# martenlienen/generative-turbulence

Hardware: AMD Instinct MI355X
Metric: U-Net fwd+bwd voxels/sec (DDPM training step, 192x64x48x4) (higher is better)
Workload: dtype bf16

## Files before the change

generative-turbulence_amd/csrc/tdx_conv3.h:

```cpp
#pragma once
#include "tdx_common.h"

struct Conv3Geom {
    int B;
    int Xi, Yi, Zi;
    int Xo, Yo, Zo;
    int off;
};

bool conv3_mfma_supported(int C1, int C2, int Cout);
bool conv3_mfma_f32_supported(int C1, int C2, int Cout);
static inline int conv3_layout_kc(int dtype, int K, int N) {
    if (dtype == 1 || dtype == 3) return conv3_mfma_supported(K, 0, N) ? 16 : 0;
    return conv3_mfma_f32_supported(K, 0, N) ? 8 : 0;
}
static inline bool conv3_uses_mfma_layout(int dtype, int K, int N) { return (dtype == 1 || dtype == 3) && conv3_mfma_supported(K, 0, N); }
bool conv3_mfma_split_supported(int C1, int C2, int Cout);

struct Conv3Ext {
    int ld1, ld2;
    const void* init;
    bool init_shared;
};

// ... 45 lines not shown

int conv3_mfma_launch(const Conv3Call& c);
int conv3_mfma_split_launch(const Conv3Call& c);
int conv3_mfma_f32_launch(const Conv3Call& c);
int conv3_direct_launch(const Conv3Call& c);
int conv3_fold_launch(const Conv3Call& c);

int conv3_ring_depth(int C1, int C2, int N, int B, int X, int Y, int Z, bool data_gradient);
int conv3_ring_launch(const Conv3Call& c, int depth);

bool conv3_small_plan(Conv3SmallPlan& p, int C1, int C2, int N, int B, int X, int Y, int Z, bool data_gradient, bool split);
int conv3_small_launch(const Conv3Call& c, const Conv3SmallPlan& p);

struct Conv3WgradCall {
    const void* x1; int C1;
    const void* x2; int C2;
    const void* dy;
    float* dwp;
    float* dbias;
    int B, X, Y, Z, Cout;
    hipStream_t st;
    float* slabs; int max_slabs; int* nslab;
    bool hf;
};
bool tdx_deterministic();
static inline float* conv3_wgrad_merge(const Conv3WgradCall& c, int& nsplit, int64_t& slab_stride) {
    if (tdx_deterministic() && c.slabs != nullptr && nsplit > c.max_slabs) nsplit = c.max_slabs > 0 ? c.max_slabs : 1;
    const bool use_slabs = c.slabs != nullptr && nsplit <= c.max_slabs;
    slab_stride = use_slabs ? (int64_t)27 * (c.C1 + c.C2) * c.Cout : 0;
    if (c.nslab) *c.nslab = use_slabs ? nsplit : 0;
    return use_slabs ? c.slabs : c.dwp;
}
bool conv3_wgrad_mfma_supported(int C1, int C2, int Cout);
bool conv3_wgrad_mfma_split_supported(int C1, int C2, int Cout);
bool conv3_wgrad_mfma_f32_supported(int C1, int C2, int Cout);
int conv3_wgrad_mfma_launch(const Conv3WgradCall& c);
int conv3_wgrad_small_launch(const Conv3WgradCall& c);
int conv3_wgrad_ring_launch(const Conv3WgradCall& c);
int conv3_wgrad_mfma_split_launch(const Conv3WgradCall& c);
int conv3_wgrad_split_ring_launch(const Conv3WgradCall& c);
int conv3_wgrad_mfma_f32_launch(const Conv3WgradCall& c);
int conv3_wgrad_direct_launch(const Conv3WgradCall& c, int dtype);
int conv3_unpack_wgrad_launch(const Conv3WgradCall& c, float* dw, float* dbw, float* dbias, bool many);
int tdx_persistent_cus();
int ordered_sum_launch(const float* slabs, int nslab, int64_t stride, float* dst, int rows, int cols, int64_t ld, bool add,
                       hipStream_t st);
size_t bias_grad_ordered_scratch_floats(int C);
int bias_grad_ordered_launch(const void* dy, int64_t nvox, int C, int dtype, float* dbias, float* part, size_t part_floats,
                             hipStream_t st);
void* tdx_scratch_ptr();
size_t tdx_scratch_bytes();

size_t conv3_shell_buffer_bytes(int B, int X, int Y, int Z, int N);
int conv3_shell_launch(const void* dy, const void* wb, void* d1, int D1, void* d2, int B, int X, int Y, int Z, int K, int N,
                       int mode, hipStream_t st, void* sbuf = nullptr);

#define TDX_GN_REPLICAS 32
int gn_finalize_launch(double* acc, float* stats, int B, int C, int G, int64_t V, float eps, int replicas,
                       hipStream_t st);
int gn_stats_launch(const void* x, float* stats, int B, int64_t V, int C, int G, float eps, int dtype, void* workspace,
                    bool clean, hipStream_t stream);
```

generative-turbulence_amd/csrc/tdx_conv3_entry.hip:

```cpp
#include "tdx_common.h"
#include "tdx_conv3.h"
#include <stdlib.h>
#include <algorithm>

int tdx_persistent_cus() {
    const char* env = getenv("TDX_PERSISTENT_CUS");
    int n = env ? atoi(env) : 256;
    n = n < 8 ? 8 : (n > 256 ? 256 : n);
    return n & ~7;
}
static void* g_scratch = nullptr;
static size_t g_scratch_bytes = 0;
void* tdx_scratch_ptr() { return g_scratch; }
size_t tdx_scratch_bytes() { return g_scratch_bytes; }
extern "C" int tdx_set_scratch(void* ptr, size_t bytes) {
    if (ptr != nullptr && bytes < 64) return TDX_EINVAL;
    g_scratch = ptr;
    g_scratch_bytes = ptr ? bytes : 0;
    return TDX_OK;
}

Conv3Route conv3_route(int dtype, int impl, int C1, int C2, int N, int B, int X, int Y, int Z, bool data_gradient) {
    Conv3Route r;
    r.fmt = dtype; r.family = TDX_KERNEL_DIRECT; r.status = TDX_OK; r.ring_depth = 0;
// ... 144 lines not shown
                                      const void* add1, const void* add2, int B, int X, int Y, int Z, int Cout, int dtype,
                                      int impl, void* workspace, void* stream) {
    return conv3_bwd_data_impl(dy, wb, dx1, C1, dx2, C2, add1, add2, B, X, Y, Z, Cout, dtype, impl, workspace, stream);
}

#define W3_MAX_SLABS 8
static int w3_slab_capacity(int Cin, int Cout) {
    const int64_t c = ((int64_t)1 << 19) / ((int64_t)Cin * Cout);
    return (int)(c < W3_MAX_SLABS ? W3_MAX_SLABS : (c > 512 ? 512 : c));
}
extern "C" size_t tdx_conv3_bwd_weight_workspace_bytes(int Cin, int Cout, int impl) {
    (void)impl;
    return (size_t)(1 + w3_slab_capacity(Cin, Cout)) * 27 * Cin * Cout * sizeof(float) + (size_t)Cout * sizeof(float) + 512;
}

struct Conv3WgradRoute {
    int (*launch)(const Conv3WgradCall&);
    bool f32;
    int status;
};
static Conv3WgradRoute conv3_wgrad_route(int dtype, int impl, int C1, int C2, int Cout) {
    if (dtype == TDX_F32 && impl == TDX_CONV_SPLIT && conv3_wgrad_mfma_split_supported(C1, C2, Cout))
        return {conv3_wgrad_mfma_split_launch, true, TDX_OK};
    if (dtype == TDX_F32 && impl != TDX_CONV_DIRECT && conv3_wgrad_mfma_f32_supported(C1, C2, Cout))
        return {conv3_wgrad_mfma_f32_launch, true, TDX_OK};
    if (impl == TDX_CONV_MFMA || (impl == TDX_CONV_AUTO && tdx_is_h16(dtype) && conv3_wgrad_mfma_supported(C1, C2, Cout))) {
        if (!tdx_is_h16(dtype)) return {nullptr, false, TDX_EDTYPE};
        if (!conv3_wgrad_mfma_supported(C1, C2, Cout)) return {nullptr, false, TDX_ESHAPE};
        return {conv3_wgrad_mfma_launch, false, TDX_OK};
    }
    return {nullptr, false, TDX_OK};
}

extern "C" int tdx_conv3_bwd_weight(const void* x1, int C1, const void* x2, int C2, const void* dy, float* dw,
                                    float* dbias, int B, int X, int Y, int Z, int Cout, int dtype, int impl,
                                    void* workspace, void* stream) {
    TDX_CHECK_ARG(x1 && dy && dw && workspace && B > 0 && X > 0 && Y > 0 && Z > 0 && C1 > 0 && C2 >= 0 && Cout > 0);
    TDX_CHECK_ARG(C2 == 0 || x2);
    const int Cin = C1 + C2;
    if ((C1 % 8) || (C2 % 8) || (Cout % 8)) return TDX_ESHAPE;
    hipStream_t st = as_stream(stream);
    const bool clean = (impl & TDX_WS_CLEAN) != 0;
    float* dwp = (float*)workspace;
    float* dbw = dwp + (size_t)27 * Cin * Cout;
    if (!clean) {
        int e = tdx_zero_async(dwp, ((size_t)27 * Cin * Cout + Cout) * sizeof(float), st);
        if (e != TDX_OK) return e;
    }
    const Conv3WgradRoute r = conv3_wgrad_route(dtype, impl & 0xff, C1, C2, Cout);
    if (r.status != TDX_OK) return r.status;
    int nslab = 0;
    const bool det = tdx_deterministic();
    float* slab_base = dbw + ((Cout + 63) / 64) * 64;
    auto ordered_bias = [&]() -> int {
        if (!det || !dbias) return TDX_OK;
        return bias_grad_ordered_launch(dy, (int64_t)B * X * Y * Z, Cout, dtype, dbias, slab_base,
                                        (size_t)W3_MAX_SLABS * 27 * Cin * Cout, st);
    };
    Conv3WgradCall c = {x1, C1, x2, C2, dy, dwp, (dbias && !det) ? dbw : nullptr, B, X, Y, Z, Cout, st, slab_base, 0, &nslab,
                        dtype == TDX_F16};
    if (r.launch != nullptr) {
        c.max_slabs = (r.f32 && !det) ? W3_MAX_SLABS : w3_slab_capacity(Cin, Cout);
    } else if (det) {
        c.max_slabs = std::min(w3_slab_capacity(Cin, Cout), 64);
    }
    const int rc = r.launch != nullptr ? r.launch(c) : conv3_wgrad_direct_launch(c, dtype);
// ... 5 lines not shown
```

generative-turbulence_amd/csrc/tdx_conv3_wgrad_mfma.hip:

```cpp
#include "tdx_conv3_wgrad.h"
#include <stdlib.h>

typedef WgradBrick<4> W3;
#define W3_NSTEPS (W3::NVOX / 16)
#define W3_TAPS_PER_WAVE 7

bool conv3_wgrad_mfma_supported(int C1, int C2, int Cout) {
    const bool c1_ok = (C1 % 32) == 0 || (C2 == 0 && (C1 % 16) == 0);
    return C1 > 0 && c1_ok && (C2 % 32) == 0 && (Cout % 32) == 0;
}

#ifdef W3_STAMPS
#define W3_NSTAMP 64
__device__ unsigned long long* w3_stamps_dev;
#define W3_T()                                                                              \
    do {                                                                                    \
        if (it_ >= 4 && it_ < 12) {                                                         \
            const unsigned long long t_ = __builtin_amdgcn_s_memtime();                     \
            if (lane == 0 && nst_ < W3_NSTAMP) sStamp_[wave * W3_NSTAMP + nst_] = t_;       \
            ++nst_;                                                                         \
        }                                                                                   \
    } while (0)
#else
#define W3_T() do { } while (0)
// ... 188 lines not shown
#endif

    const int r = lane & 31, hh = lane >> 5;
#pragma unroll
    for (int t = 0; t < W3_TAPS_PER_WAVE; ++t) {
        const int ltap = wave + 4 * t;
        if (ltap < 27) {
            const int tap = wgrad_global_tap(gv, ltap);
#pragma unroll
            for (int nt = 0; nt < NT; ++nt)
#pragma unroll
                for (int i = 0; i < 16; ++i) {
                    const int ci = ci0 + (i & 3) + 8 * (i >> 2) + 4 * hh;
                    if (ci >= Cin) continue;
                    float* dst = &dwp[((int64_t)tap * Cin + ci) * Cout + co0 + nt * 32 + r];
                    if (slab_stride) dst[(int64_t)split * slab_stride] = acc[t][nt][i];
                    else atomicAdd(dst, acc[t][nt][i]);
                }
        }
    }
    if (do_bias) {
        __syncthreads();
        float* red = reinterpret_cast<float*>(smem);
#pragma unroll
        for (int e = 0; e < 8; ++e) red[tid * 8 + e] = bs[e];
        __syncthreads();
        if (tid < 32 * NT) {
            const int q8 = tid >> 3, e = tid & 7;
            float t = 0.f;
            for (int k = q8; k < 256; k += 4 * NT) t += red[k * 8 + e];
            atomicAdd(&dbias[co0 + tid], t);
        }
    }
}

int conv3_wgrad_mfma_launch(const Conv3WgradCall& c) {
    const int Cout = c.Cout;
    {
        int rs = conv3_wgrad_small_launch(c);
        if (rs != TDX_ESHAPE) return rs;
#ifndef W3_STAMPS
        rs = conv3_wgrad_ring_launch(c);
        if (rs != TDX_ESHAPE) return rs;
#endif
    }
    const int Cin = c.C1 + c.C2;
    const int NT = (Cout % 64 == 0) ? 2 : 1;
    static const bool no_perm = getenv("TDX_CONV3_PERM") && atoi(getenv("TDX_CONV3_PERM")) == 0;
    WgradView g;
    const int nbricks = conv3_wgrad_view(g, c, W3::BX, W3::BY, W3::BZ, !no_perm);
    const int n_ci = (Cin + 31) / 32, n_co = Cout / (32 * NT);
    const int ntiles = n_ci * n_co;
    int nsplit = ((NT == 2 ? 256 : 512) + ntiles - 1) / ntiles;
    if (nsplit > nbricks) nsplit = nbricks;
    if (nsplit < 1) nsplit = 1;
    int64_t slab_stride;
    float* out = conv3_wgrad_merge(c, nsplit, slab_stride);
    size_t lds = W3::XBYTES + (size_t)NT * W3::GPLANE;
#ifdef W3_STAMPS
    lds += 4 * W3_NSTAMP * 8;
#endif
    dim3 grid((unsigned)(ntiles * nsplit));
#define W3_LAUNCH(NTV, HFV)                                                                                          \
    do {                                                                                                             \
        auto kern = conv3_wgrad_mfma_kernel<NTV, HFV>;                                                                  \
        hipError_t e = hipFuncSetAttribute((const void*)kern, hipFuncAttributeMaxDynamicSharedMemorySize, (int)lds); \
// ... 10 lines not shown
```

generative-turbulence_amd/csrc/tdx_conv3_wgrad_ring.hip:

```cpp
#include "tdx_conv3_wgrad.h"
#include <stdlib.h>
#include <algorithm>
#include <type_traits>

typedef WgradBrick<4> WR;
#define WR_NSTEPS (WR::NVOX / 16)
#define WR_XPIECES ((WR::NHALO * 4 + 63) / 64)
#define WR_XBUF (WR_XPIECES * 1024)
#define WR_XPW ((WR_XPIECES + 3) / 4)
#define WR_CW 8
#define WR_GBUF(NTN) ((NTN) * WR::GPLANE)
#define WR_GPW(NTN) (4 * (NTN))
#define WR_SLOTS(NTN) ((NTN) == 2 ? 7 : 4)

template <int NTN, bool HF>
__global__ void __launch_bounds__(768, 3)
conv3_wgrad_ring_kernel(const bf16* __restrict__ x1, int C1, const bf16* __restrict__ x2, int C2, const bf16* __restrict__ dy,
                        float* __restrict__ dwp, float* __restrict__ dbias, WgradView gv, int Cout, int nsplit, int n_ci_tiles,
                        int64_t slab_stride, const void* __restrict__ zeros) {
    extern __shared__ __attribute__((aligned(1024))) unsigned char smem[];
    unsigned char* sX = smem;
    unsigned char* sG = smem + 2 * WR_XBUF;
    constexpr int GBUF = WR_GBUF(NTN), GPW = WR_GPW(NTN), SLOTS = WR_SLOTS(NTN);
    const unsigned lds0 = lds_addr(smem);
// ... 159 lines not shown
                step(2 * s2 + 1, 1);
            }
        }
    };
    if (NTN == 2 ? odd : (cnt == 4 || bias_slot)) run(std::true_type{}); else run(std::false_type{});

    const int r = lane & 31, hh = lane >> 5;
#pragma unroll
    for (int i = 0; i < SLOTS; ++i) {
        const int T = first + i;
        if (i < cnt) {
            const int ltap = T / NTN, nt = T % NTN;
            const int tap = wgrad_global_tap(gv, ltap);
#pragma unroll
            for (int e = 0; e < 16; ++e) {
                const int ci = ci0 + (e & 3) + 8 * (e >> 2) + 4 * hh;
                if (ci >= Cin) continue;
                float* dst = &dwp[((int64_t)tap * Cin + ci) * Cout + co0 + nt * 32 + r];
                if (slab_stride) dst[(int64_t)split * slab_stride] = acc[i][e];
                else atomicAdd(dst, acc[i][e]);
            }
        } else if (bias_slot && i == SLOTS - 1 && dbias != nullptr && ci0 == 0 && hh == 0) {
            atomicAdd(&dbias[co0 + (NTN == 2 ? (wave - 6) * 32 : 0) + r], acc[i][0]);
        }
    }
}

bool conv3_wgrad_ring_supported(int C1, int C2, int Cout) {
    const char* env = getenv("TDX_WGRAD_RING");
    if (env && atoi(env) == 0) return false;
    return conv3_wgrad_mfma_supported(C1, C2, Cout) && (Cout % 32) == 0 && tdx_scratch_ptr() != nullptr && tdx_scratch_bytes() >= 16;
}

int conv3_wgrad_ring_launch(const Conv3WgradCall& c) {
    const int Cout = c.Cout;
    if (!conv3_wgrad_ring_supported(c.C1, c.C2, Cout)) return TDX_ESHAPE;
    const int Cin = c.C1 + c.C2;
    WgradView g;
    const int nbricks = conv3_wgrad_view(g, c, WR::BX, WR::BY, WR::BZ);
    const int NTN = (Cout % 64) == 0 ? 2 : 1;
    {
        const char* env = getenv("TDX_WGRAD_RING");
        if (NTN == 1 && env && atoi(env) == 2) return TDX_ESHAPE;
    }
    const int n_ci = (Cin + 31) / 32, n_co = Cout / (32 * NTN);
    const int ntiles = n_ci * n_co;
    const int cus = tdx_persistent_cus();
    int nsplit = cus >= 256 ? (256 + ntiles - 1) / ntiles : std::max(cus / ntiles, 1);
    if (nsplit > nbricks) nsplit = nbricks;
    if (nsplit < 1) nsplit = 1;
    if (nbricks < 4 * nsplit) return TDX_ESHAPE;
    const size_t lds = (size_t)2 * WR_XBUF + (size_t)2 * WR_GBUF(NTN);
    int64_t slab_stride;
    float* out = conv3_wgrad_merge(c, nsplit, slab_stride);
    static bool attr_set[2][2] = {{false, false}, {false, false}};
#define WR_GO(NTNV, HFV)                                                                                                          \
    do {                                                                                                                          \
        auto kern = conv3_wgrad_ring_kernel<NTNV, HFV>;                                                                           \
        if (!attr_set[NTNV - 1][HFV]) {                                                                                           \
            hipError_t e = hipFuncSetAttribute((const void*)kern, hipFuncAttributeMaxDynamicSharedMemorySize, (int)lds);          \
            if (e != hipSuccess) return (int)e;                                                                                   \
            attr_set[NTNV - 1][HFV] = true;                                                                                       \
        }                                                                                                                         \
        hipLaunchKernelGGL(kern, dim3((unsigned)(ntiles * nsplit)), dim3(768), lds, c.st, (const bf16*)c.x1, c.C1,                \
                           (const bf16*)c.x2, c.C2, (const bf16*)c.dy, out, c.dbias, g, Cout, nsplit, n_ci, slab_stride,          \
                           tdx_scratch_ptr());                                                                                    \
    } while (0)
    if (NTN == 2) { if (c.hf) WR_GO(2, true); else WR_GO(2, false); }
    else { if (c.hf) WR_GO(1, true); else WR_GO(1, false); }
#undef WR_GO
    return tdx_launch_status();
}
```

generative-turbulence_amd/csrc/tdx_conv3_wgrad_small.hip:

```cpp
#include "tdx_conv3_wgrad.h"
#include <stdlib.h>

#define WS_MAXROWS 256
#define WS_TAPS_PER_WAVE 7

struct WsGeom {
    int B, E[3];
    int nbg;
    int xs, gx;
    int Ix, Iy, Iz;
    int ngroups;
    int xbytes;
    int grows;
};

template <int NT, bool HF>
__global__ void __launch_bounds__(256, 1)
conv3_wgrad_small_kernel(const bf16* __restrict__ x1, int C1, const bf16* __restrict__ x2, int C2, const bf16* __restrict__ dy,
                         float* __restrict__ dwp, float* __restrict__ dbias, WsGeom g, int Cout, int nsplit, int n_ci_tiles,
                         int64_t slab_stride) {
    extern __shared__ __attribute__((aligned(16))) unsigned char smem[];
    const int gbytes = NT * g.grows * 64;
    unsigned char* sX = smem;
    unsigned char* sG = smem + 2 * g.xbytes;
// ... 136 lines not shown
            if (s + 1 < nsteps) {
                read_a(s3, A0);
                read_b(s2, B0);
                mfma_step(A1, B1);
                __builtin_amdgcn_sched_group_barrier(0x008, 1, 0);
                __builtin_amdgcn_sched_group_barrier(0x100, NRD, 0);
                __builtin_amdgcn_sched_group_barrier(0x008, NMF - 1, 0);
            }
        }
    }

    const int r = lane & 31, hh = lane >> 5;
#pragma unroll
    for (int t = 0; t < WS_TAPS_PER_WAVE; ++t) {
        const int tap = wave + 4 * t;
        if (tap < 27) {
#pragma unroll
            for (int nt = 0; nt < NT; ++nt)
#pragma unroll
                for (int i = 0; i < 16; ++i) {
                    const int ci = ci0 + (i & 3) + 8 * (i >> 2) + 4 * hh;
                    float* dst = &dwp[((int64_t)tap * Cin + ci) * Cout + co0 + nt * 32 + r];
                    if (slab_stride) dst[(int64_t)split * slab_stride] = acc[t][nt][i];
                    else atomicAdd(dst, acc[t][nt][i]);
                }
        }
    }
    if (do_bias && ones_slot && hh == 0) {
#pragma unroll
        for (int nt = 0; nt < NT; ++nt) atomicAdd(&dbias[co0 + nt * 32 + r], acc[WS_TAPS_PER_WAVE - 1][nt][0]);
    }
}

int conv3_wgrad_small_launch(const Conv3WgradCall& c) {
    const int B = c.B, X = c.X, Y = c.Y, Z = c.Z, Cout = c.Cout;
    static const int mode = getenv("TDX_WGRAD_SMALL") ? atoi(getenv("TDX_WGRAD_SMALL")) : 1;
    if (mode == 0) return TDX_ESHAPE;
    const int Cin = c.C1 + c.C2;
    if ((c.C1 % 32) || (c.C2 % 32) || (Cout % 32) || Cin < 128) return TDX_ESHAPE;
    const char* env_rows = getenv("TDX_WGRAD_SMALL_ROWS");
    const int64_t rows_total = (int64_t)B * X * Y * Z;
    if (rows_total > (env_rows ? atoi(env_rows) : 8000)) return TDX_ESHAPE;
    WsGeom g;
    g.B = B; g.E[0] = X; g.E[1] = Y; g.E[2] = Z;
    const int plane = Y * Z, V = X * plane;
    if (plane > WS_MAXROWS) return TDX_ESHAPE;
    if (V <= WS_MAXROWS) { g.nbg = std::min(B, WS_MAXROWS / V); g.xs = X; g.gx = 1; }
    else { g.nbg = 1; g.xs = WS_MAXROWS / plane; g.gx = ceil_div(X, g.xs); }
    g.Ix = g.xs + 2; g.Iy = Y + 2; g.Iz = Z + 2;
    const int NT = (Cout % 64 == 0) ? 2 : 1;
    auto sizes = [&]() {
        const int entries = g.nbg * g.Ix * g.Iy * g.Iz;
        g.xbytes = ((entries * 64 + 1023) >> 10) << 10;
        g.grows = ((g.nbg * g.xs * plane + 15) >> 4) << 4;
        return (size_t)2 * g.xbytes + (size_t)2 * NT * g.grows * 64 + (WS_MAXROWS + (g.xbytes >> 6)) * sizeof(unsigned);
    };
    size_t lds = sizes();
    while (lds > 160 * 1024 && (g.nbg > 1 || g.xs > 1)) {
        if (g.nbg > 1) --g.nbg; else { --g.xs; g.gx = ceil_div(X, g.xs); g.Ix = g.xs + 2; }
        lds = sizes();
    }
    if (lds > 160 * 1024) return TDX_ESHAPE;
    g.ngroups = ceil_div(B, g.nbg) * g.gx;
    const int n_ci = Cin / 32, n_co = Cout / (32 * NT);
    const int ntiles = n_ci * n_co;
    int nsplit = std::max(1, std::min(g.ngroups, ceil_div(256, ntiles)));
    int64_t slab_stride;
    float* out = conv3_wgrad_merge(c, nsplit, slab_stride);
    dim3 grid((unsigned)(ntiles * nsplit));
#define WS_LAUNCH(NTV, HFV)                                                                                           \
    do {                                                                                                              \
        auto kern = conv3_wgrad_small_kernel<NTV, HFV>;                                                               \
        static size_t attr = 0;                                                                                       \
        if (lds > attr) {                                                                                             \
            hipError_t e = hipFuncSetAttribute((const void*)kern, hipFuncAttributeMaxDynamicSharedMemorySize, (int)lds); \
            if (e != hipSuccess) return (int)e;                                                                       \
            attr = lds;                                                                                               \
        }                                                                                                             \
        hipLaunchKernelGGL(kern, grid, dim3(256), lds, c.st, (const bf16*)c.x1, c.C1, (const bf16*)c.x2, c.C2,        \
                           (const bf16*)c.dy, out, c.dbias, g, Cout, nsplit, n_ci, slab_stride);                      \
    } while (0)
    if (NT == 2) { if (c.hf) WS_LAUNCH(2, true); else WS_LAUNCH(2, false); }
    else { if (c.hf) WS_LAUNCH(1, true); else WS_LAUNCH(1, false); }
#undef WS_LAUNCH
    return tdx_launch_status();
}
```

generative-turbulence_amd/turbdiff_amd/_lib.py:

```python

from __future__ import annotations

import ctypes as C
import os
import threading
from pathlib import Path

import torch

_HERE = Path(__file__).resolve().parent
LIB_PATH = Path(os.environ.get("TDX_LIB", _HERE / "libtdx_hip.so"))

F32, BF16 = 0, 1
F16 = 3
CONV_AUTO, CONV_DIRECT, CONV_MFMA, CONV_SPLIT = 0, 1, 2, 3
F32_SPLIT = 2
WS_CLEAN = 0x100

_vp, _i, _i64, _u64, _f, _sz = C.c_void_p, C.c_int, C.c_int64, C.c_uint64, C.c_float, C.c_size_t

SIGNATURES = {
    "tdx_version": (_i, []),
    "tdx_arch": (C.c_char_p, []),
    "tdx_set_scratch": (_i, [_vp, _sz]),
    "tdx_ncv_to_nvc": (_i, [_vp, _vp, _i, _i, _i64, _i, _i, _vp]),
    "tdx_nvc_to_ncv": (_i, [_vp, _vp, _i, _i, _i64, _i, _i, _vp]),
    "tdx_cast": (_i, [_vp, _vp, _i64, _i, _i, _vp]),
    "tdx_conv3_pack_weight": (_i, [_vp, _vp, _vp, _i, _i, _i, _vp]),
    "tdx_conv3_pack_weights": (_i, [_vp, _i, _i, _vp]),
    "tdx_transpose_many": (_i, [_vp, _i, _vp]),
    "tdx_conv3_fwd": (_i, [_vp, _i, _vp, _i, _vp, _vp, _vp, _i, _i, _i, _i, _i, _i, _i, _vp]),
    "tdx_conv3_uses_ring": (_i, [_i] * 7),
    "tdx_conv3_ring_brick_depth": (_i, [_i] * 7),
    "tdx_conv3_fwd_kernel": (_i, [_i] * 9),
    "tdx_conv3_fwd_gn": (_i, [_vp, _i, _vp, _i, _vp, _vp, _vp, _vp, _i, _f, _vp, _i, _i, _i, _i, _i, _i, _i, _vp]),
    "tdx_conv3_fwd_partial": (_i, [_vp, _i, _i, _vp, _vp, _vp, _i, _vp, _vp, _i, _f, _vp, _i, _i, _i, _i, _i, _i, _i, _vp]),
    "tdx_conv3_bwd_data_workspace_bytes": (_sz, [_i, _i, _i, _i, _i, _i, _i]),
    "tdx_conv3_bwd_data": (_i, [_vp, _vp, _vp, _i, _vp, _i, _i, _i, _i, _i, _i, _i, _i, _i, _vp, _vp]),
    "tdx_conv3_bwd_data_add": (_i, [_vp, _vp, _vp, _i, _vp, _i, _vp, _vp, _i, _i, _i, _i, _i, _i, _i, _vp, _vp]),
    "tdx_conv3_bwd_weight_workspace_bytes": (_sz, [_i, _i, _i]),
    "tdx_conv3_bwd_weight": (_i, [_vp, _i, _vp, _i, _vp, _vp, _vp, _i, _i, _i, _i, _i, _i, _i, _vp, _vp]),
    "tdx_conv1_fwd": (_i, [_vp, _i, _vp, _i, _vp, _i, _vp, _vp, _vp, _i64, _i, _i, _vp]),
    "tdx_conv1_fwd_gn": (_i, [_vp, _i, _vp, _i, _vp, _i, _vp, _vp, _vp, _vp, _vp, _i, _vp, _i, _i64, _i, _i, _vp]),
    "tdx_conv1_bwd_weight": (_i, [_vp, _i, _vp, _i, _vp, _i, _vp, _i64, _i, _vp]),
    "tdx_conv1_bwd_weight_oc": (_i, [_vp, _i, _vp, _i, _vp, _i, _vp, _i, _i64, _i, _vp]),
    "tdx_encode_fwd": (_i, [_vp, _i, _vp, _vp, _vp, _i, _vp, _vp, _vp, _i, _i64, _i, _i, _vp]),
    "tdx_encode_bwd": (_i, [_vp, _vp, _i, _vp, _i, _vp, _vp, _vp, _vp, _vp, _vp, _i, _i64, _i, _i, _vp]),
    "tdx_decode_fwd": (_i, [_vp, _vp, _vp, _vp, _i, _i64, _i, _i, _i, _vp]),
    "tdx_decode_bwd": (_i, [_vp, _vp, _vp, _vp, _vp, _vp, _i, _i64, _i, _i, _i, _vp]),
    "tdx_gn_workspace_bytes": (_sz, [_i, _i]),
    "tdx_gn_stats": (_i, [_vp, _vp, _i, _i64, _i, _i, _f, _i, _vp, _vp]),
    "tdx_gn_apply": (_i, [_vp, _vp, _vp, _vp, _vp, _vp, _vp, _vp, _i, _i64, _i, _i, _i, _i, _vp]),
    "tdx_gn_apply_decode": (_i, [_vp, _vp, _vp, _vp, _vp, _vp, _vp, _vp, _i, _i64, _i, _i, _i, _i, _vp]),
    "tdx_gn_apply_encoded": (_i, [_vp, _vp, _vp, _vp, _vp, _i, _vp, _vp, _vp, _i, _vp, _vp, _vp, _i, _i64, _i, _i, _i, _vp]),
    "tdx_gn_bwd": (_i, [_vp] * 12 + [_i, _i64, _i, _i, _i, _i, _vp, _vp]),
    "tdx_resize_fwd": (_i, [_vp, _vp] + [_i] * 9 + [_vp]),
    "tdx_resize_bwd": (_i, [_vp, _vp, _vp] + [_i] * 9 + [_vp]),
    "tdx_attn_fwd": (_i, [_vp, _vp, _vp, _i, _i, _i, _i, _i, _vp]),
    "tdx_attn_bwd": (_i, [_vp, _vp, _vp, _vp, _vp, _i, _i, _i, _i, _i, _vp, _vp]),
    "tdx_attn_bwd_workspace_bytes": (_sz, [_i, _i, _i, _i]),
    "tdx_cell_mask": (_i, [_vp, _i64, _vp, _i64, _vp]),
    "tdx_q_sample": (_i, [_vp, _vp, _vp, _vp, _vp, _i, _vp, _i, _vp, _i, _i, _i64, _vp]),
    "tdx_p_sample_step": (_i, [_vp] * 7 + [_i, _vp, _i, _i, _vp, _i, _i, _i64, _vp]),
    "tdx_p_sample_step_rng": (_i, [_vp] * 5 + [_i, _vp, _i, _i, _vp, _i, _i, _i64, _u64, _vp, _vp, _vp]),
    "tdx_p_sample_step_lv": (_i, [_vp] * 8 + [_i, _vp, _i, _i, _vp, _i, _i, _i64, _vp]),
    "tdx_p_sample_step_lv_rng": (_i, [_vp] * 6 + [_i, _vp, _i, _i, _vp, _i, _i, _i64, _u64, _vp, _vp, _vp]),
    "tdx_ddim_step": (_i, [_vp] * 7 + [_i, _vp, _vp, _vp, _i, _i, _vp, _i, _i, _i64, _vp]),
    "tdx_ddim_step_rng": (_i, [_vp] * 5 + [_i, _vp, _vp, _vp, _i, _i, _vp, _i, _i, _i64, _u64, _vp, _vp, _vp]),
    "tdx_masked_loss": (_i, [_vp, _vp, _vp, _i64, _i, _vp, _vp, _i, _i, _i64, _vp, _vp]),
    "tdx_masked_loss_dyn": (_i, [_vp, _vp, _vp, _vp, _i, _vp, _vp, _i, _i, _i64, _vp, _vp]),
    "tdx_masked_loss_workspace_bytes": (_sz, []),
    "tdx_elbo_loss": (_i, [_vp] * 5 + [_i64, _vp, _vp, _vp, _i, _i, _i, _i, C.c_double, _vp, _vp, _i, _i, _i64, _vp, _vp]),
    "tdx_elbo_loss_dyn": (_i, [_vp] * 5 + [_vp, _vp, _vp, _vp, _i, _i, _i, _i, C.c_double, _vp, _vp, _i, _i, _i64, _vp, _vp]),
    "tdx_elbo_loss_workspace_bytes": (_sz, []),
# ... 247 lines not shown


def _launch(name, args, work, meta):
    t = TIMER
    if t is not None and name in t.names:
        s, e = torch.cuda.Event(enable_timing=True), torch.cuda.Event(enable_timing=True)
        s.record()
        rc = getattr(load(), name)(*args)
        e.record()
        t.records.append((name, s, e, work, meta() if callable(meta) else meta))
        return rc
    return getattr(load(), name)(*args)


def query(name: str, *args) -> int:
    return int(getattr(load(), name)(*args))


def kernel_sources_fingerprint(pattern: str = "tdx_conv*") -> str | None:
    import hashlib

    src = _HERE.parent / "csrc"
    files = sorted(f for f in src.glob(pattern) if f.suffix in (".hip", ".h"))
    if not files:
        return None
    h = hashlib.sha256()
    for f in files:
        h.update(f.name.encode())
        h.update(f.read_bytes())
    return h.hexdigest()[:16]


KERNEL_DIRECT, KERNEL_BRICK, KERNEL_SMALL, KERNEL_RING = 0, 1, 2, 3


def conv3_fwd_meta(C1, C2, Cout, B, X, Y, Z, dt, real=None):
    es = 2 if dt in H16_DTYPES else 4
    cin = real or (C1 + C2)
    return {"kind": query("tdx_conv3_fwd_kernel", C1, C2, Cout, B, X, Y, Z, dtype_code(dt), conv_impl()),
            "bytes": float((cin + Cout) * B * X * Y * Z * es + 27 * cin * Cout * es)}
```

include/tdx.h:

```cpp
#ifndef TDX_H
#define TDX_H

#include <stddef.h>
#include <stdint.h>

#ifdef __cplusplus
extern "C" {
#endif

#define TDX_F32 0
#define TDX_BF16 1

#define TDX_OK 0
#define TDX_EINVAL (-1)
#define TDX_ESHAPE (-2)
#define TDX_EDTYPE (-3)

#define TDX_CONV_AUTO 0
#define TDX_CONV_DIRECT 1
#define TDX_CONV_MFMA 2
#define TDX_CONV_SPLIT 3
#define TDX_F32_SPLIT 2
#define TDX_F16 3
#define TDX_WS_CLEAN 0x100
// ... 21 lines not shown
} TdxTransposeJob;
int tdx_transpose_many(const TdxTransposeJob* jobs, int n, void* stream);

int tdx_conv3_fwd(const void* x1, int C1, const void* x2, int C2, const void* wf, const float* bias, void* y,
                  int B, int X, int Y, int Z, int Cout, int dtype, int impl, void* stream);

int tdx_conv3_uses_ring(int C1, int C2, int Cout, int B, int X, int Y, int Z);
int tdx_conv3_ring_brick_depth(int C1, int C2, int Cout, int B, int X, int Y, int Z);
#define TDX_KERNEL_DIRECT 0
#define TDX_KERNEL_BRICK 1
#define TDX_KERNEL_SMALL 2
#define TDX_KERNEL_RING 3
int tdx_conv3_fwd_kernel(int C1, int C2, int Cout, int B, int X, int Y, int Z, int dtype, int impl);

int tdx_conv3_fwd_gn(const void* x1, int C1, const void* x2, int C2, const void* wf, const float* bias, void* y,
                     float* stats, int G, float eps, void* gn_workspace, int B, int X, int Y, int Z, int Cout,
                     int dtype, int impl, void* stream);

int tdx_conv3_fwd_partial(const void* x1, int C1, int ld1, const void* wf, const float* bias, const void* init,
                          int init_shared, void* y, float* stats, int G, float eps, void* gn_workspace, int B, int X,
                          int Y, int Z, int Cout, int dtype, int impl, void* stream);

size_t tdx_conv3_bwd_data_workspace_bytes(int B, int X, int Y, int Z, int Cin, int dtype, int impl);
int tdx_conv3_bwd_data(const void* dy, const void* wb, void* dx1, int C1, void* dx2, int C2, int accumulate,
                       int B, int X, int Y, int Z, int Cout, int dtype, int impl, void* workspace, void* stream);

int tdx_conv3_bwd_data_add(const void* dy, const void* wb, void* dx1, int C1, void* dx2, int C2, const void* add1,
                           const void* add2, int B, int X, int Y, int Z, int Cout, int dtype, int impl,
                           void* workspace, void* stream);

size_t tdx_conv3_bwd_weight_workspace_bytes(int Cin, int Cout, int impl);
int tdx_conv3_bwd_weight(const void* x1, int C1, const void* x2, int C2, const void* dy, float* dw, float* dbias,
                         int B, int X, int Y, int Z, int Cout, int dtype, int impl, void* workspace, void* stream);

int tdx_conv1_fwd(const void* x1, int C1, const void* x2, int C2, const float* w, int ldw, const float* bias,
                  const void* add, void* y, int64_t rows, int Cout, int dtype, void* stream);
int tdx_conv1_fwd_gn(const void* x1, int C1, const void* x2, int C2, const float* w, int ldw, const float* bias,
                     const void* h, const float* stats, const float* gamma, const float* beta, int groups, void* y,
                     int B, int64_t V, int Cout, int dtype, void* stream);
int tdx_conv1_bwd_weight(const void* x, int Cin, const void* dy, int Cout, float* dw, int ldw, float* dbias,
                         int64_t rows, int dtype, void* stream);
int tdx_conv1_bwd_weight_oc(const void* x, int Cin, const void* dy, int Cout, float* dw, int ldw, float* dbias,
                            int accumulate, int64_t rows, int dtype, void* stream);

int tdx_encode_fwd(const float* x, int Fx, const float* wx, const float* bx, const float* c, int Fc, const float* wc,
                   const float* bc, void* y, int B, int64_t V, int D, int dtype, void* stream);
int tdx_encode_bwd(const void* dy, const float* x, int Fx, const float* c, int Fc, const float* wc, float* dwx,
                   float* dbx, float* dwc, float* dbc, float* dc, int B, int64_t V, int D, int dtype, void* stream);
int tdx_decode_fwd(const void* h, const float* w, const float* bias, float* y, int B, int64_t V, int D, int F, int dtype,
                   void* stream);
int tdx_decode_bwd(const float* dy, const void* h, const float* w, void* dh, float* dw, float* db, int B, int64_t V, int D,
                   int F, int dtype, void* stream);

size_t tdx_gn_workspace_bytes(int B, int C);
int tdx_gn_stats(const void* x, float* stats, int B, int64_t V, int C, int G, float eps, int dtype, void* workspace,
                 void* stream);
int tdx_gn_apply(const void* x, const float* stats, const float* gamma, const float* beta, const float* scale,
                 const float* shift, const void* res, void* y, int B, int64_t V, int C, int G, int act, int dtype,
                 void* stream);
int tdx_gn_apply_encoded(const void* x, const float* stats, const float* gamma, const float* beta, const float* x_raw, int Fx,
                         const float* wx, const float* bx, const float* c_raw, int Fc, const float* wc, const float* bc,
                         void* y, int B, int64_t V, int D, int G, int dtype, void* stream);
int tdx_gn_apply_decode(const void* x, const float* stats, const float* gamma, const float* beta, const void* res,
                        const float* w, const float* bias, float* out, int B, int64_t V, int C, int G, int F, int dtype,
                        void* stream);
int tdx_gn_bwd(const void* x, const void* dy, const float* stats, const float* gamma, const float* beta,
// ... 180 lines not shown
```

Before: 169.5 million.

## Add specialized ring wgrad kernel for 16-input-channel 3D convolutions

Adds a dedicated persistent weight-gradient kernel for the Cin=16 case (first U-Net layer). It uses warp-specialized loader waves that DMA halo bricks into double-buffered LDS and compute waves that pack taps two per MFMA tile, and it folds the bias gradient into the padded tap slot. The ring launcher now routes C1=16 layers to this kernel. The previous generic ring padded Cin to 32, so this is meant to remove the wasted half of the MFMA work and LDS traffic. Plan and introspection helpers are also refactored out so the chosen kernel can be queried.

```diff
diff --git a/generative-turbulence_amd/csrc/tdx_conv3.h b/generative-turbulence_amd/csrc/tdx_conv3.h
--- a/generative-turbulence_amd/csrc/tdx_conv3.h
+++ b/generative-turbulence_amd/csrc/tdx_conv3.h
@@ -101,11 +101,17 @@
     return use_slabs ? c.slabs : c.dwp;
 }
 bool conv3_wgrad_mfma_supported(int C1, int C2, int Cout);
+bool conv3_wgrad_ring_supported(int C1, int C2, int Cout);
 bool conv3_wgrad_mfma_split_supported(int C1, int C2, int Cout);
 bool conv3_wgrad_mfma_f32_supported(int C1, int C2, int Cout);
 int conv3_wgrad_mfma_launch(const Conv3WgradCall& c);
 int conv3_wgrad_small_launch(const Conv3WgradCall& c);
 int conv3_wgrad_ring_launch(const Conv3WgradCall& c);
+bool conv3_wgrad_c16_case(int C1, int C2, int Cout);
+int conv3_wgrad_c16_launch(const Conv3WgradCall& c);
+bool conv3_wgrad_small_case(const Conv3WgradCall& c);
+int conv3_wgrad_ring_kind(const Conv3WgradCall& c);
+int conv3_wgrad_mfma_kind(const Conv3WgradCall& c);
 int conv3_wgrad_mfma_split_launch(const Conv3WgradCall& c);
 int conv3_wgrad_split_ring_launch(const Conv3WgradCall& c);
 int conv3_wgrad_mfma_f32_launch(const Conv3WgradCall& c);
diff --git a/generative-turbulence_amd/csrc/tdx_conv3_entry.hip b/generative-turbulence_amd/csrc/tdx_conv3_entry.hip
--- a/generative-turbulence_amd/csrc/tdx_conv3_entry.hip
+++ b/generative-turbulence_amd/csrc/tdx_conv3_entry.hip
@@ -200,6 +200,15 @@
     return {nullptr, false, TDX_OK};
 }
 
+extern "C" int tdx_conv3_bwd_weight_kernel(int C1, int C2, int Cout, int B, int X, int Y, int Z, int dtype, int impl) {
+    const Conv3WgradRoute r = conv3_wgrad_route(dtype, impl & 0xff, C1, C2, Cout);
+    if (r.launch == nullptr) return TDX_KERNEL_DIRECT;
+    if (r.f32) return TDX_KERNEL_BRICK;
+    Conv3WgradCall c = {};
+    c.C1 = C1; c.C2 = C2; c.Cout = Cout; c.B = B; c.X = X; c.Y = Y; c.Z = Z;
+    return conv3_wgrad_mfma_kind(c);
+}
+
 extern "C" int tdx_conv3_bwd_weight(const void* x1, int C1, const void* x2, int C2, const void* dy, float* dw,
                                     float* dbias, int B, int X, int Y, int Z, int Cout, int dtype, int impl,
                                     void* workspace, void* stream) {
diff --git a/generative-turbulence_amd/csrc/tdx_conv3_wgrad_mfma.hip b/generative-turbulence_amd/csrc/tdx_conv3_wgrad_mfma.hip
--- a/generative-turbulence_amd/csrc/tdx_conv3_wgrad_mfma.hip
+++ b/generative-turbulence_amd/csrc/tdx_conv3_wgrad_mfma.hip
@@ -244,6 +244,12 @@
             atomicAdd(&dbias[co0 + tid], t);
         }
     }
+}
+
+int conv3_wgrad_mfma_kind(const Conv3WgradCall& c) {
+    if (conv3_wgrad_small_case(c)) return TDX_KERNEL_SMALL;
+    const int ring = conv3_wgrad_ring_kind(c);
+    return ring >= 0 ? ring : TDX_KERNEL_BRICK;
 }
 
 int conv3_wgrad_mfma_launch(const Conv3WgradCall& c) {
diff --git a/generative-turbulence_amd/csrc/tdx_conv3_wgrad_ring.hip b/generative-turbulence_amd/csrc/tdx_conv3_wgrad_ring.hip
--- a/generative-turbulence_amd/csrc/tdx_conv3_wgrad_ring.hip
+++ b/generative-turbulence_amd/csrc/tdx_conv3_wgrad_ring.hip
@@ -215,24 +215,43 @@
     return conv3_wgrad_mfma_supported(C1, C2, Cout) && (Cout % 32) == 0 && tdx_scratch_ptr() != nullptr && tdx_scratch_bytes() >= 16;
 }
 
-int conv3_wgrad_ring_launch(const Conv3WgradCall& c) {
+struct WrPlan {
+    WgradView g;
+    int NTN, n_ci, ntiles, nsplit;
+};
+static bool wr_plan(const Conv3WgradCall& c, WrPlan& p) {
     const int Cout = c.Cout;
-    if (!conv3_wgrad_ring_supported(c.C1, c.C2, Cout)) return TDX_ESHAPE;
+    if (!conv3_wgrad_ring_supported(c.C1, c.C2, Cout)) return false;
     const int Cin = c.C1 + c.C2;
-    WgradView g;
-    const int nbricks = conv3_wgrad_view(g, c, WR::BX, WR::BY, WR::BZ);
-    const int NTN = (Cout % 64) == 0 ? 2 : 1;
+    const int nbricks = conv3_wgrad_view(p.g, c, WR::BX, WR::BY, WR::BZ);
+    p.NTN = (Cout % 64) == 0 ? 2 : 1;
     {
         const char* env = getenv("TDX_WGRAD_RING");
-        if (NTN == 1 && env && atoi(env) == 2) return TDX_ESHAPE;
-    }
-    const int n_ci = (Cin + 31) / 32, n_co = Cout / (32 * NTN);
-    const int ntiles = n_ci * n_co;
+        if (p.NTN == 1 && env && atoi(env) == 2) return false;
+    }
+    p.n_ci = (Cin + 31) / 32;
+    p.ntiles = p.n_ci * (Cout / (32 * p.NTN));
     const int cus = tdx_persistent_cus();
-    int nsplit = cus >= 256 ? (256 + ntiles - 1) / ntiles : std::max(cus / ntiles, 1);
+    int nsplit = cus >= 256 ? (256 + p.ntiles - 1) / p.ntiles : std::max(cus / p.ntiles, 1);
     if (nsplit > nbricks) nsplit = nbricks;
     if (nsplit < 1) nsplit = 1;
-    if (nbricks < 4 * nsplit) return TDX_ESHAPE;
+    p.nsplit = nsplit;
+    return nbricks >= 4 * nsplit;
+}
+
+int conv3_wgrad_ring_kind(const Conv3WgradCall& c) {
+    if (conv3_wgrad_c16_case(c.C1, c.C2, c.Cout)) return TDX_KERNEL_RING_C16;
+    WrPlan p;
+    return wr_plan(c, p) ? TDX_KERNEL_RING : -1;
+}
+
+int conv3_wgrad_ring_launch(const Conv3WgradCall& c) {
+    if (conv3_wgrad_c16_case(c.C1, c.C2, c.Cout)) return conv3_wgrad_c16_launch(c);
+    WrPlan p;
+    if (!wr_plan(c, p)) return TDX_ESHAPE;
+    const int Cout = c.Cout, NTN = p.NTN, n_ci = p.n_ci, ntiles = p.ntiles;
+    const WgradView& g = p.g;
+    int nsplit = p.nsplit;
     const size_t lds = (size_t)2 * WR_XBUF + (size_t)2 * WR_GBUF(NTN);
     int64_t slab_stride;
     float* out = conv3_wgrad_merge(c, nsplit, slab_stride);
diff --git a/generative-turbulence_amd/csrc/tdx_conv3_wgrad_ring_c16.hip b/generative-turbulence_amd/csrc/tdx_conv3_wgrad_ring_c16.hip
--- /dev/null
+++ b/generative-turbulence_amd/csrc/tdx_conv3_wgrad_ring_c16.hip
@@ -0,0 +1,221 @@
+#include "tdx_conv3_wgrad.h"
+#include <stdlib.h>
+#include <algorithm>
+#include <type_traits>
+
+typedef WgradBrick<4, 32> WC;
+typedef WgradBrick<4> WCG;
+#define WC_NSTEPS (WC::NVOX / 16)
+#define WC_XPIECES ((WC::NHALO * 2 + 63) / 64)
+#define WC_XBUF (WC_XPIECES * 1024)
+#define WC_XPW ((WC_XPIECES + 3) / 4)
+#define WC_CW 8
+#define WC_GBUF (2 * WCG::GPLANE)
+#define WC_GPW 8
+#define WC_SLOTS 4
+
+typedef __attribute__((ext_vector_type(4))) unsigned wc_u32x4;
+
+template <bool HF>
+__global__ void __launch_bounds__(768, 3)
+conv3_wgrad_c16_kernel(const bf16* __restrict__ x, const bf16* __restrict__ dy, float* __restrict__ dwp,
+                       float* __restrict__ dbias, WgradView gv, int Cout, int nsplit, int64_t slab_stride,
+                       const void* __restrict__ zeros) {
+    extern __shared__ __attribute__((aligned(1024))) unsigned char smem[];
+    unsigned char* sX = smem;
+    unsigned char* sG = smem + 2 * WC_XBUF;
+    const unsigned lds0 = lds_addr(smem);
+
+    const int tid = threadIdx.x, lane = tid & 63;
+    const int wave = __builtin_amdgcn_readfirstlane(tid >> 6);
+    constexpr int Cin = 16;
+    const int tile = blockIdx.x / nsplit, split = blockIdx.x - tile * nsplit;
+    const int co0 = tile * 64;
+    const int nbricks = gv.B * gv.nb[0] * gv.nb[1] * gv.nb[2];
+
+    if (wave >= WC_CW) {
+        const int lw = wave - WC_CW;
+        int xh[WC_XPW];
+#pragma unroll
+        for (int i = 0; i < WC_XPW; ++i) {
+            const int pc = min(min(lw * WC_XPW + i, WC_XPIECES - 1) * 64 + lane, WC::NHALO * 2 - 1);
+            const int hv = pc >> 1, q2 = pc & 1;
+            int hx, hy, hz;
+            WC::halo_coords(hv, hx, hy, hz);
+            xh[i] = hx | (hy << 8) | (hz << 16) | (q2 << 24);
+        }
+        const int g_plane = (lw * WC_GPW) / 16, g_p0 = (lw * WC_GPW) % 16;
+        const int g_e0 = g_p0 * 64 + lane;
+        auto issue = [&](int brick, int buf) {
+            int bx, by, bz;
+            const int bb = wgrad_brick_coords(gv, brick, bx, by, bz);
+#pragma unroll
+            for (int i = 0; i < WC_XPW; ++i) {
+                const int sx = min(max(bx * WC::BX + (xh[i] & 0xff) - 1, 0), gv.E[0] - 1);
+                const int sy = min(max(by * WC::BY + ((xh[i] >> 8) & 0xff) - 1, 0), gv.E[1] - 1);
+                const int sz = min(max(bz * WC::BZ + ((xh[i] >> 16) & 0xff) - 1, 0), gv.E[2] - 1);
+                const int64_t vox = (int64_t)bb * gv.batch + sx * gv.s[0] + sy * gv.s[1] + sz * gv.s[2];
+                lds_dma16(x + vox * Cin + ((xh[i] >> 24) & 1) * 8, lds0 + buf * WC_XBUF + min(lw * WC_XPW + i, WC_XPIECES - 1) * 1024);
+            }
+#pragma unroll
+            for (int j = 0; j < WC_GPW; ++j) {
+                const int e = g_e0 + 64 * j, v = e >> 2, c4 = e & 3;
+                const int vx = bx * WC::BX + (v >> 6), vy = by * WC::BY + ((v >> 3) & 7), vz = bz * WC::BZ + (v & 7);
+                const bool ok = vx < gv.E[0] && vy < gv.E[1] && vz < gv.E[2];
+                const int64_t vox = wgrad_voxel(gv, bb, min(vx, gv.E[0] - 1), min(vy, gv.E[1] - 1), min(vz, gv.E[2] - 1));
+                const bf16* src = ok ? dy + vox * Cout + co0 + g_plane * 32 + c4 * 8 : reinterpret_cast<const bf16*>(zeros);
+                lds_dma16(src, lds0 + 2 * WC_XBUF + buf * WC_GBUF + g_plane * WCG::GPLANE + (g_p0 + j) * 1024);
+            }
+        };
+        int brick = split, it = 0;
+        if (brick < nbricks) issue(brick, 0);
+        for (; brick < nbricks; brick += nsplit, ++it) {
+            asm volatile("s_waitcnt vmcnt(0)" ::: "memory");
+            lds_barrier();
+            if (brick + nsplit < nbricks) issue(brick + nsplit, (it + 1) & 1);
+        }
+        asm volatile("s_waitcnt vmcnt(0)" ::: "memory");
+        return;
+    }
+
+    const int first = wave < 4 ? 4 * wave : 16 + 3 * (wave - 4);
+    const int cnt = wave < 4 ? 4 : 3;
+    const int mt0 = first >> 1;
+    const bool odd = (first & 1) != 0;
+    const bool last = wave == WC_CW - 1;
+
+    const WgradLane L = wgrad_lane(lane);
+    const int half = (lane >> 4) & 1;
+    int a_off[2];
+#pragma unroll
+    for (int a = 0; a < 2; ++a)
+        a_off[a] = wgrad_x_frag_row<WC>(L, WC::tap_offset(min(2 * (mt0 + a) + half, 26))) * 32 + (lane & 3) * 8;
+    const int b_row = (8 * L.kh + L.q) * 64 + L.col_off;
+
+    f32x16 acc[WC_SLOTS];
+#pragma unroll
+    for (int i = 0; i < WC_SLOTS; ++i)
+#pragma unroll
+        for (int e = 0; e < 16; ++e) acc[i][e] = 0.f;
+    const wc_u32x4 ones = __builtin_bit_cast(wc_u32x4, H16<HF>::ones());
+
+    auto run = [&](auto cnt_c, auto odd_c, auto last_c) {
+        constexpr int CNT = decltype(cnt_c)::value;
+        constexpr int ODD = decltype(odd_c)::value ? 1 : 0;
+        constexpr bool LAST = decltype(last_c)::value;
+        int it = 0;
+        for (int brick = split; brick < nbricks; brick += nsplit, ++it) {
+            lds_barrier();
+            const unsigned char* bX = sX + (it & 1) * WC_XBUF;
+            const unsigned char* bG = sG + (it & 1) * WC_GBUF + b_row;
+            auto read_a = [&](int s, int a) {
+                const unsigned char* ap = bX + a_off[a] + ((s >> 2) * WC::HY + 2 * (s & 3)) * WC::HZ * 32;
+                return tr_frag(ap, ap + 4 * 32);
+            };
+            auto operand_a = [&](bf16x8 f, int a) {
+                if (LAST && a == 1) {
+                    wc_u32x4 u = __builtin_bit_cast(wc_u32x4, f);
+#pragma unroll
+                    for (int k = 0; k < 4; ++k) u[k] = half ? ones[k] : u[k];
+                    f = __builtin_bit_cast(bf16x8, u);
+                }
+                return f;
+            };
+            auto read_b = [&](int s, int nt) {
+                const unsigned char* bp = bG + nt * WCG::GPLANE + s * (16 * 64);
+                return tr_frag(bp, bp + 4 * 64);
+            };
+            bf16x8 A[2][2], Bq[2][2];
+#pragma unroll
+            for (int a = 0; a < 2; ++a) A[0][a] = read_a(0, a);
+#pragma unroll
+            for (int nt = 0; nt < 2; ++nt) Bq[0][nt] = read_b(0, nt);
+
+            auto step = [&](int s, int cur) {
+                const int sn = min(s + 1, WC_NSTEPS - 1), nx = cur ^ 1;
+#pragma unroll
+                for (int a = 0; a < 2; ++a) A[nx][a] = read_a(sn, a);
+#pragma unroll
+                for (int nt = 0; nt < 2; ++nt) Bq[nx][nt] = read_b(sn, nt);
+                const bf16x8 Au[2] = {A[cur][0], operand_a(A[cur][1], 1)};
+#pragma unroll
+                for (int i = 0; i < CNT; ++i) {
+                    const int T = ODD + i;
+                    acc[i] = H16<HF>::mfma(Au[T >> 1], Bq[cur][T & 1], acc[i]);
+                }
+                __builtin_amdgcn_sched_group_barrier(0x100, CNT == 4 ? 2 : 4, 0); __builtin_amdgcn_sched_group_barrier(0x008, 1, 0);
+                __builtin_amdgcn_sched_group_barrier(0x100, 2, 0); __builtin_amdgcn_sched_group_barrier(0x008, 1, 0);
+                __builtin_amdgcn_sched_group_barrier(0x100, 2, 0); __builtin_amdgcn_sched_group_barrier(0x008, 1, 0);
+                if constexpr (CNT == 4) {
+                    __builtin_amdgcn_sched_group_barrier(0x100, 2, 0); __builtin_amdgcn_sched_group_barrier(0x008, 1, 0);
+                }
+            };
+#pragma unroll 1
+            for (int s2 = 0; s2 < WC_NSTEPS / 2; ++s2) {
+                step(2 * s2, 0);
+                step(2 * s2 + 1, 1);
+            }
+        }
+    };
+    using T_ = std::true_type;
+    using F_ = std::false_type;
+    if (cnt == 4) run(std::integral_constant<int, 4>{}, F_{}, F_{});
+    else if (!odd) run(std::integral_constant<int, 3>{}, F_{}, F_{});
+    else if (!last) run(std::integral_constant<int, 3>{}, T_{}, F_{});
+    else run(std::integral_constant<int, 3>{}, T_{}, T_{});
+
+    const int r = lane & 31, hh = lane >> 5;
+#pragma unroll
+    for (int i = 0; i < WC_SLOTS; ++i) {
+        if (i >= cnt) continue;
+        const int T = first + i, mt = T >> 1, nt = T & 1;
+#pragma unroll
+        for (int e = 0; e < 16; ++e) {
+            const int ltap = 2 * mt + (e >> 3);
+            if (ltap > 26) {
+                if (e == 8 && hh == 0 && dbias != nullptr) atomicAdd(&dbias[co0 + nt * 32 + r], acc[i][e]);
+                continue;
+            }
+            const int tap = wgrad_global_tap(gv, ltap);
+            const int ci = (e & 3) + 8 * ((e >> 2) & 1) + 4 * hh;
+            float* dst = &dwp[((int64_t)tap * Cin + ci) * Cout + co0 + nt * 32 + r];
+            if (slab_stride) dst[(int64_t)split * slab_stride] = acc[i][e];
+            else atomicAdd(dst, acc[i][e]);
+        }
+    }
+}
+
+bool conv3_wgrad_c16_case(int C1, int C2, int Cout) {
+    const char* env = getenv("TDX_WGRAD_C16");
+    if (env && atoi(env) == 0) return false;
+    return C1 == 16 && C2 == 0 && (Cout % 64) == 0 && conv3_wgrad_ring_supported(C1, C2, Cout);
+}
+
+int conv3_wgrad_c16_launch(const Conv3WgradCall& c) {
+    const int Cout = c.Cout;
+    if (!conv3_wgrad_c16_case(c.C1, c.C2, Cout)) return TDX_ESHAPE;
+    WgradView g;
+    const int nbricks = conv3_wgrad_view(g, c, WC::BX, WC::BY, WC::BZ);
+    const int ntiles = Cout / 64;
+    const int cus = tdx_persistent_cus();
+    int nsplit = cus >= 256 ? (256 + ntiles - 1) / ntiles : std::max(cus / ntiles, 1);
+    nsplit = std::max(std::min(nsplit, nbricks / 2), 1);
+    const size_t lds = (size_t)2 * WC_XBUF + (size_t)2 * WC_GBUF;
+    int64_t slab_stride;
+    float* out = conv3_wgrad_merge(c, nsplit, slab_stride);
+    static bool attr_set[2] = {false, false};
+#define WC_GO(HFV)                                                                                                        \
+    do {                                                                                                                  \
+        auto kern = conv3_wgrad_c16_kernel<HFV>;                                                                          \
+        if (!attr_set[HFV]) {                                                                                             \
+            hipError_t e = hipFuncSetAttribute((const void*)kern, hipFuncAttributeMaxDynamicSharedMemorySize, (int)lds);  \
+            if (e != hipSuccess) return (int)e;                                                                           \
+            attr_set[HFV] = true;                                                                                         \
+        }                                                                                                                 \
+        hipLaunchKernelGGL(kern, dim3((unsigned)(ntiles * nsplit)), dim3(768), lds, c.st, (const bf16*)c.x1,              \
+                           (const bf16*)c.dy, out, c.dbias, g, Cout, nsplit, slab_stride, tdx_scratch_ptr());             \
+    } while (0)
+    if (c.hf) WC_GO(true); else WC_GO(false);
+#undef WC_GO
+    return tdx_launch_status();
+}
diff --git a/generative-turbulence_amd/csrc/tdx_conv3_wgrad_small.hip b/generative-turbulence_amd/csrc/tdx_conv3_wgrad_small.hip
--- a/generative-turbulence_amd/csrc/tdx_conv3_wgrad_small.hip
+++ b/generative-turbulence_amd/csrc/tdx_conv3_wgrad_small.hip
@@ -192,19 +192,18 @@
     }
 }
 
-int conv3_wgrad_small_launch(const Conv3WgradCall& c) {
+static bool ws_plan(const Conv3WgradCall& c, WsGeom& g, size_t& lds) {
     const int B = c.B, X = c.X, Y = c.Y, Z = c.Z, Cout = c.Cout;
     static const int mode = getenv("TDX_WGRAD_SMALL") ? atoi(getenv("TDX_WGRAD_SMALL")) : 1;
-    if (mode == 0) return TDX_ESHAPE;
+    if (mode == 0) return false;
     const int Cin = c.C1 + c.C2;
-    if ((c.C1 % 32) || (c.C2 % 32) || (Cout % 32) || Cin < 128) return TDX_ESHAPE;
+    if ((c.C1 % 32) || (c.C2 % 32) || (Cout % 32) || Cin < 128) return false;
     const char* env_rows = getenv("TDX_WGRAD_SMALL_ROWS");
     const int64_t rows_total = (int64_t)B * X * Y * Z;
-    if (rows_total > (env_rows ? atoi(env_rows) : 8000)) return TDX_ESHAPE;
-    WsGeom g;
+    if (rows_total > (env_rows ? atoi(env_rows) : 8000)) return false;
     g.B = B; g.E[0] = X; g.E[1] = Y; g.E[2] = Z;
     const int plane = Y * Z, V = X * plane;
-    if (plane > WS_MAXROWS) return TDX_ESHAPE;
+    if (plane > WS_MAXROWS) return false;
     if (V <= WS_MAXROWS) { g.nbg = std::min(B, WS_MAXROWS / V); g.xs = X; g.gx = 1; }
     else { g.nbg = 1; g.xs = WS_MAXROWS / plane; g.gx = ceil_div(X, g.xs); }
     g.Ix = g.xs + 2; g.Iy = Y + 2; g.Iz = Z + 2;
@@ -215,13 +214,27 @@
         g.grows = ((g.nbg * g.xs * plane + 15) >> 4) << 4;
         return (size_t)2 * g.xbytes + (size_t)2 * NT * g.grows * 64 + (WS_MAXROWS + (g.xbytes >> 6)) * sizeof(unsigned);
     };
-    size_t lds = sizes();
+    lds = sizes();
     while (lds > 160 * 1024 && (g.nbg > 1 || g.xs > 1)) {
         if (g.nbg > 1) --g.nbg; else { --g.xs; g.gx = ceil_div(X, g.xs); g.Ix = g.xs + 2; }
         lds = sizes();
     }
-    if (lds > 160 * 1024) return TDX_ESHAPE;
+    if (lds > 160 * 1024) return false;
     g.ngroups = ceil_div(B, g.nbg) * g.gx;
+    return true;
+}
+bool conv3_wgrad_small_case(const Conv3WgradCall& c) {
+    WsGeom g;
+    size_t lds;
+    return ws_plan(c, g, lds);
+}
+
+int conv3_wgrad_small_launch(const Conv3WgradCall& c) {
+    WsGeom g;
+    size_t lds;
+    if (!ws_plan(c, g, lds)) return TDX_ESHAPE;
+    const int Cin = c.C1 + c.C2, Cout = c.Cout;
+    const int NT = (Cout % 64 == 0) ? 2 : 1;
     const int n_ci = Cin / 32, n_co = Cout / (32 * NT);
     const int ntiles = n_ci * n_co;
     int nsplit = std::max(1, std::min(g.ngroups, ceil_div(256, ntiles)));
diff --git a/generative-turbulence_amd/turbdiff_amd/_lib.py b/generative-turbulence_amd/turbdiff_amd/_lib.py
--- a/generative-turbulence_amd/turbdiff_amd/_lib.py
+++ b/generative-turbulence_amd/turbdiff_amd/_lib.py
@@ -40,6 +40,7 @@
     "tdx_conv3_bwd_data_add": (_i, [_vp, _vp, _vp, _i, _vp, _i, _vp, _vp, _i, _i, _i, _i, _i, _i, _i, _vp, _vp]),
     "tdx_conv3_bwd_weight_workspace_bytes": (_sz, [_i, _i, _i]),
     "tdx_conv3_bwd_weight": (_i, [_vp, _i, _vp, _i, _vp, _vp, _vp, _i, _i, _i, _i, _i, _i, _i, _vp, _vp]),
+    "tdx_conv3_bwd_weight_kernel": (_i, [_i] * 9),
     "tdx_conv1_fwd": (_i, [_vp, _i, _vp, _i, _vp, _i, _vp, _vp, _vp, _i64, _i, _i, _vp]),
     "tdx_conv1_fwd_gn": (_i, [_vp, _i, _vp, _i, _vp, _i, _vp, _vp, _vp, _vp, _vp, _i, _vp, _i, _i64, _i, _i, _vp]),
     "tdx_conv1_bwd_weight": (_i, [_vp, _i, _vp, _i, _vp, _i, _vp, _i64, _i, _vp]),
@@ -353,6 +354,7 @@
 
 
 KERNEL_DIRECT, KERNEL_BRICK, KERNEL_SMALL, KERNEL_RING = 0, 1, 2, 3
+KERNEL_RING_C16 = 4
 
 
 def conv3_fwd_meta(C1, C2, Cout, B, X, Y, Z, dt, real=None):
diff --git a/include/tdx.h b/include/tdx.h
--- a/include/tdx.h
+++ b/include/tdx.h
@@ -77,6 +77,8 @@
 size_t tdx_conv3_bwd_weight_workspace_bytes(int Cin, int Cout, int impl);
 int tdx_conv3_bwd_weight(const void* x1, int C1, const void* x2, int C2, const void* dy, float* dw, float* dbias,
                          int B, int X, int Y, int Z, int Cout, int dtype, int impl, void* workspace, void* stream);
+#define TDX_KERNEL_RING_C16 4
+int tdx_conv3_bwd_weight_kernel(int C1, int C2, int Cout, int B, int X, int Y, int Z, int dtype, int impl);
 
 int tdx_conv1_fwd(const void* x1, int C1, const void* x2, int C2, const float* w, int ldw, const float* bias,
                   const void* add, void* y, int64_t rows, int Cout, int dtype, void* stream);
```

Result: no change. 167.7 million (median of 2 runs) (-1.1%).
